# nirschl-lab/stain2stain

Measured on AMD Instinct MI355X. Metric: paired 256x256 stain tiles/sec (full CFM optimisation step), higher is better.
Workload: dtype bf16

## Files before the change

include/stain2stain_hip.h:

```cpp
#ifndef STAIN2STAIN_HIP_H
#define STAIN2STAIN_HIP_H

#ifdef __cplusplus
extern "C" {
#endif

#define S2S_OK 0
#define S2S_ERR_SHAPE (-1)
#define S2S_ERR_ALIGN (-2)
#define S2S_ERR_DTYPE (-3)
#define S2S_ERR_LAUNCH (-4)
#define S2S_ERR_NULL (-5)

#define S2S_BF16 0
#define S2S_F32 1

int s2s_conv3x3_stat_blocks(int dtype, int B, int H, int W, int Cout);
int s2s_conv3x3_nhwc(int dtype, const void* x0, int ld0, int c0, const void* x1, int ld1, int c1,
                     const void* w_packed, const float* bias, void* y, int ldy, float* stat_part,
                     const float* ep_scale, const float* ep_shift, int relu, int B, int H, int W, int Cout,
                     void* stream);

int s2s_conv3x3_ksplit(int dtype, int B, int H, int W, int Cout, int cin);
int s2s_conv3x3_nhwc_k(int dtype, const void* x0, int ld0, int c0, const void* x1, int ld1, int c1,
                       const void* w_packed, const float* bias, void* y, int ldy, float* stat_part,
                       const float* ep_scale, const float* ep_shift, int relu, float* kwork, int B, int H, int W,
                       int Cout, void* stream);
int s2s_conv3x3_stat_rows(int dtype, int B, int H, int W, int Cout, int c0, int c1, int ld0, int ld1, int has_bias);
int s2s_conv3x3_staged(int dtype, int B, int H, int W, int Cout, int c0, int c1, int ld0, int ld1, int ldy, int stats);
int s2s_conv3x3_family(int dtype, int B, int H, int W, int Cout, int c0, int c1, int ld0, int ld1, int ldy, int has_bias,
                       int has_affine, int stats, int stat_rows, int kwork);
int s2s_conv3x3_nhwc_s(int dtype, const void* x0, int ld0, int c0, const void* x1, int ld1, int c1, const void* w_packed,
                       const float* bias, void* y, int ldy, float* stat_part, int stat_rows, const float* ep_scale,
                       const float* ep_shift, int relu, float* kwork, int B, int H, int W, int Cout, void* stream);
int s2s_debug_conv_clock(long* out_host, int n);

int s2s_conv3x3_wgrad_splits(int dtype, int B, int H, int W, int Cin, int Cout);
int s2s_conv3x3_wgrad_nhwc(int dtype, const void* dy, int lddy, int Cout, const void* x0, int ld0, int c0,
                           const void* x1, int ld1, int c1, float* part, float* grad_oihw, int accumulate,
                           int B, int H, int W, void* stream);
int s2s_conv3x3_wgrad_phase(int dtype, const void* dy, int lddy, int Cout, const void* x0, int ld0, int c0,
                            const void* x1, int ld1, int c1, float* part, float* grad_oihw, int accumulate,
                            int B, int H, int W, int phases, void* stream);

int s2s_stem_stat_blocks(int B, int H, int W);
int s2s_stem_conv3x3_fwd(int dtype, const float* x_nchw, const float* w_oihw, const float* bias, void* y, int ldy,
                         float* stat_part, int B, int H, int W, int Cin, int Cout, void* stream);
int s2s_stem_wgrad_blocks(int B, int H, int W);
int s2s_stem_conv3x3_wgrad(int dtype, const void* dy, int lddy, const float* x_nchw, float* part, float* dw_oihw,
                           float* dbias, int accumulate, int B, int H, int W, int Cin, int Cout, void* stream);
int s2s_head_conv1x1_fwd(int dtype, const void* x, int ldx, const float* w, const float* bias, float* y_nchw, int B,
                         int H, int W, int C, int Cout, void* stream);
int s2s_head_wgrad_blocks(int B, int H, int W);
int s2s_head_conv1x1_bwd(int dtype, const float* dy_nchw, const void* x, int ldx, const float* w, void* dx, int lddx,
                         float* part, float* dw, float* dbias, int accumulate, int B, int H, int W, int C, int Cout,
                         void* stream);

int s2s_head_loss_blocks(int B, int H, int W);
int s2s_head_loss_fused(int dtype, const void* x, int ldx, const float* w, const float* bias, const float* u_nchw,
                        float* v_nchw, void* dx, int lddx, float grad_scale, float* part, double* lpart, float* dw,
                        float* dbias, float* loss, int accumulate, int B, int H, int W, int C, int Cout, void* stream);

int s2s_tail_blocks(int B, int H, int W);
int s2s_tail_fwd_loss(int dtype, const void* raw, int ldx, const float* scale, const float* shift, const float* mean,
                      const float* invstd, const float* w, const float* bias, const float* u_nchw, float* v_nchw,
                      float* g_nchw, float grad_scale, float* part, double* lpart, float* bnwork, float* dw,
                      float* dbias, float* loss, float* dgamma, float* dbeta, float* conv_dbias, int accumulate, int B,
                      int H, int W, int C, int Cout, void* stream);
int s2s_tail_bwd_apply(int dtype, const void* raw, int ldx, const float* g_nchw, const float* w, const float* scale,
                       const float* shift, const float* mean, const float* invstd, const float* gamma,
                       const float* bnwork, void* dx, int lddx, int B, int H, int W, int C, int Cout, void* stream);

int s2s_bn_finalize(const float* part, int nblk, int C, long count, const float* gamma, const float* beta,
                    float* running_mean, float* running_var, long* num_batches_tracked, float momentum, float eps,
                    float* mean, float* invstd, float* scale, float* shift, void* stream);
int s2s_bn_finalize_b(const float* part, int nblk, int C, long count, const float* gamma, const float* beta,
                      float* running_mean, float* running_var, long* num_batches_tracked, float momentum, float eps,
                      float* mean, float* invstd, float* scale, float* shift, const float* conv_bias, void* stream);
int s2s_bn_eval_prepare(int C, const float* gamma, const float* beta, const float* running_mean,
                        const float* running_var, float eps, float* scale, float* shift, void* stream);
int s2s_bn_relu_apply(int dtype, const void* x, int ldx, const float* scale, const float* shift, void* y, int ldy,
                      void* pool, int ldp, int B, int H, int W, int C, void* stream);
int s2s_maxpool2(int dtype, const void* x, int ldx, void* pool, int ldp, int B, int H, int W, int C, void* stream);
int s2s_bn_bwd_blocks(int B, int H, int W, int C);
int s2s_bn_relu_bwd(int dtype, const void* g1, int ldg1, const void* gp, int ldgp, const float* scale,
                    const float* shift, const void* x, int ldx, const float* mean, const float* invstd, const float* gamma, float* dgamma,
                    float* dbeta, float* dbias_conv, int accumulate, void* dx, int lddx, float* work, int B, int H,
                    int W, int C, void* stream);
int s2s_bn_partial_sums(const float* part, int nblk, int C, float* sums, void* stream);
int s2s_bn_relu_bwd_phase(int dtype, const void* g1, int ldg1, const void* gp, int ldgp, const float* scale,
                          const float* shift, const void* x, int ldx, const float* mean, const float* invstd,
                          const float* gamma, float* dgamma, float* dbeta, float* dbias_conv, int accumulate, void* dx,
                          int lddx, float* work, int B, int H, int W, int C, long count_total, int phases, void* stream);

int s2s_upsample2x_bilinear_ac_fwd(int dtype, const void* x, int ldx, const float* bias_nc, void* y, int ldy, int B,
                                   int Hin, int Win, int Hout, int Wout, int C, void* stream);
int s2s_upsample2x_bilinear_ac_bwd(int dtype, const void* dy, int lddy, void* dx, int lddx, int B, int Hin, int Win,
                                   int Hout, int Wout, int C, void* stream);
int s2s_upsample2x_bilinear_ac_bwd_ref(int dtype, const void* dy, int lddy, void* dx, int lddx, int B, int Hin,
                                       int Win, int Hout, int Wout, int C, void* stream);
int s2s_upsample2x_bwd_family(int lddy, int lddx, int B, int Hin, int Win, int Hout, int Wout, int C, int reference);
int s2s_pixel_sum(int dtype, const void* x, int ldx, float* out_nc, int B, int HW, int C, int accumulate,
                  void* stream);

int s2s_time_embedding(const float* t, float* out, int B, int dim, void* stream);
int s2s_linear_fwd(const float* x, const float* w, const float* bias, float* y, int B, int K, int N, void* stream);
int s2s_linear_bwd(const float* dy, const float* x, const float* w, float* dx, float* dw, float* db, int accumulate,
                   int B, int K, int N, void* stream);
int s2s_silu_fwd(const float* h, float* a, int n, void* stream);
int s2s_silu_bwd(const float* h, const float* da, float* dh, int n, void* stream);
int s2s_cfm_sample(const float* x0, const float* x1, const float* t, const float* eps, float sigma, float* xt,
                   float* ut, int B, long per_sample, void* stream);
int s2s_mse_loss(const float* v, const float* u, float* dv, float grad_scale, float* loss, double* work, long count,
                 void* stream);
int s2s_ode_error_norm(const float* e, const float* y0, const float* y1, float atol, float rtol, float* out,
                       double* work, long n, void* stream);
int s2s_axpy(float* x, const float* y, float a, long n, void* stream);
int s2s_dp_partials(long n);
int s2s_dp_init(int phase, const float* y, const float* k1, const float* fa, double* state, double* part, float* out,
                float* t_out, int* status, float atol, float rtol, int B, long n, void* stream);
int s2s_dp_stage(int i, const float* y, const float* k1, const float* k2, const float* k3, const float* k4,
                 const float* k5, const float* k6, const double* state, float* out, float* t_out, int B, long n,
                 void* stream);
int s2s_dp_error(const float* k1, const float* k2, const float* k3, const float* k4, const float* k5, const float* k6,
                 const float* k7, const float* y, const float* y_new, const double* state, double* part, float atol,
                 float rtol, int B, long n, void* stream);
int s2s_dp_control(double* state, const double* part, int* status, int max_steps, int B, long n, void* stream);
int s2s_dp_commit(float* y, const float* y_new, float* k1, const float* k7, const double* state, int B, long n,
                  void* stream);
int s2s_rk_stage(const float* x, const float* k1, const float* k2, const float* k3, float c1, float c2, float c3, int nk,
                 float* out, float* t_out, const float* table, const int* counter, int stages, int stage, int table_len,
                 int B, long n, void* stream);
int s2s_rk_combine(float* x, const float* k1, const float* k2, const float* k3, const float* k4, float c1, float c2,
                   float c3, float c4, int nk, int* counter, int B, long n, void* stream);
int s2s_fill_f32(float* x, float v, long n, void* stream);
int s2s_euler_tick(float* t, int n, const float* table, int* counter, void* stream);

int s2s_adam_step(float* p, const float* g, float* m, float* v, long n, int step, float lr, float beta1, float beta2,
                  float eps, float weight_decay, float grad_scale, void* stream);
int s2s_adam_step_dev(float* p, const float* g, float* m, float* v, long n, const float* hyper, void* stream);
long s2s_adam_multi_blocks(long n);
int s2s_adam_multi(const void* desc, int ntensors, long total, int step, float lr, float beta1, float beta2, float eps,
                   float weight_decay, float grad_scale, void* stream);
int s2s_adam_ema_step(float* p, const float* g, float* m, float* v, float* ema, long n, int step, float lr, float beta1,
                      float beta2, float eps, float weight_decay, float grad_scale, float ema_weight, void* stream);
int s2s_adam_ema_step_dev(float* p, const float* g, float* m, float* v, float* ema, long n, const float* hyper,
                          const float* ema_weight, void* stream);
long s2s_ema_multi_blocks(long n);
int s2s_ema_multi(const void* desc, int ntensors, long total, const float* weight, void* stream);
long s2s_pack_conv3x3_fwd_elems(int Cout, int Cin);
long s2s_pack_conv3x3_dgrad_elems(int Cout, int Cin);
int s2s_pack_conv3x3(int dtype, const float* w_oihw, void* w_fwd, void* w_dgrad, int Cout, int Cin, void* stream);
int s2s_pack_conv3x3_batched(int dtype, const void* desc, int nlayers, long total, void* stream);
int s2s_nchw_to_nhwc(int dtype, const float* x_nchw, void* y, int ldy, int B, int C, int H, int W, void* stream);
int s2s_nhwc_to_nchw(int dtype, const void* x, int ldx, float* y_nchw, int accumulate, int B, int C, int H, int W,
                     void* stream);

int s2s_paired_crop_flip_normalize(const void* src_u8, const void* tgt_u8, const int* params, float* out_src,
                                   float* out_tgt, int B, int Hs, int Ws, int S, void* stream);
int s2s_pil_resize_bilinear_normalize(const void* src_u8, void* tmp_u8, const int* bounds_h, const int* kk_h,
                                      int ksize_h, const int* bounds_v, const int* kk_v, int ksize_v, void* out_u8,
                                      float* out_f, int B, int Hs, int Ws, int Ho, int Wo, void* stream);

int s2s_region_gather(const void* img_u8, long pitch, int H, int W, int band_top, int band_h, const int* origins,
                      float* out, int B, int T, void* stream);
int s2s_region_blend(const float* tiles, int c0, const float* tiles1, int c1, const int* origins, int n, int T,
                     int overlap, float* acc, int band_rows, int H, int W, int r0, int r1, void* stream);
int s2s_region_finalize(float* acc, int band_rows, int W, int C, int r0, int r1, void* out_u8, long pitch_u8,
                        float* out_f, long pitch_f, int out_top, void* stream);

int s2s_region_tissue_count(const void* img_u8, long pitch, int H, int W, int band_top, int band_h, const int* origins,
                            int n, int T, int white, int black, int* counts, void* stream);
int s2s_region_skip_weight(const int* origins, int n, int T, int overlap, float* ws, int band_rows, int H, int W,
                           int r0, int r1, void* stream);
int s2s_region_finalize_mixed(float* acc, float* ws, int band_rows, int W, int C, int r0, int r1, const void* src_u8,
                              long src_pitch, int src_top, void* out_u8, long pitch_u8, float* out_f, long pitch_f,
                              int out_top, void* stream);

int s2s_seg_loss(const float* z, const float* g, float* dz, float* out, double* work, long n, float smooth,
// ... 186 lines not shown
```

stain2stain_amd/csrc/resample.hip:

```cpp
#include "common.h"
#include <stdlib.h>

namespace {

struct Axis {
  int i0, i1;
  float w0, w1;
};

__device__ __forceinline__ Axis ac_axis(int dst, int n_in, float scale) {
  Axis a;
  const float src = scale * (float)dst;
  a.i0 = (int)src;
  if (a.i0 > n_in - 1) a.i0 = n_in - 1;
  a.i1 = a.i0 + (a.i0 < n_in - 1 ? 1 : 0);
  a.w1 = src - (float)a.i0;
  a.w0 = 1.f - a.w1;
  return a;
}

__device__ __forceinline__ int rs_pcb(int C) {
  int p = 1;
  while (p < 32 && p * 8 < C) p <<= 1;
  return p;
}

template <typename T, bool BIAS>
__global__ __launch_bounds__(256) void upsample2x_fwd_kernel(const T* __restrict__ x, int ldx,
                                                             const float* __restrict__ bias, T* __restrict__ y,
                                                             int ldy, int B, int Hin, int Win, int Hout, int Wout,
                                                             int padT, int padL, int C, int band) {
  const int cp = C >> 3;
  const int Hu = 2 * Hin, Wu = 2 * Win;
  const float sh = Hu > 1 ? (float)(Hin - 1) / (float)(Hu - 1) : 0.f;
  const float sw = Wu > 1 ? (float)(Win - 1) / (float)(Wu - 1) : 0.f;
  const int PCB = rs_pcb(C), WL = 256 / PCB;
  const int pc = threadIdx.x & (PCB - 1), slot = threadIdx.x / PCB;
  const int nrows = B * Hout;
  for (int row0 = blockIdx.x * band; row0 < nrows; row0 += gridDim.x * band)
  for (int row = row0; row < row0 + band && row < nrows; ++row) {
    const int n = row / Hout, oy = row - n * Hout;
    const int uy = oy - padT;
    const bool row_in = uy >= 0 && uy < Hu;
    const Axis ay = ac_axis(row_in ? uy : 0, Hin, sh);
    const T* const r0 = x + ((long)n * Hin + ay.i0) * Win * ldx;
    const T* const r1 = x + ((long)n * Hin + ay.i1) * Win * ldx;
    T* const yr = y + (long)row * Wout * ldy;
    for (int pb = 0; pb < cp; pb += PCB) {
      const int c8 = (pb + pc) * 8;
      if (pb + pc >= cp) continue;
      float bv[8];
#pragma unroll
      for (int k = 0; k < 8; ++k) bv[k] = BIAS ? bias[(long)n * C + c8 + k] : 0.f;
      for (int ox = slot; ox < Wout; ox += WL) {
        const int ux = ox - padL;
        f32x8 o;
        if (!row_in || ux < 0 || ux >= Wu) {
#pragma unroll
          for (int k = 0; k < 8; ++k) o.v[k] = 0.f;
        } else {
          const Axis ax = ac_axis(ux, Win, sw);
          const int o0 = ax.i0 * ldx + c8, o1 = ax.i1 * ldx + c8;
          const f32x8 v00 = load8(r0 + o0), v01 = load8(r0 + o1), v10 = load8(r1 + o0), v11 = load8(r1 + o1);
#pragma unroll
          for (int k = 0; k < 8; ++k) {
            const float b = bv[k];
            o.v[k] = ay.w0 * (ax.w0 * (v00.v[k] + b) + ax.w1 * (v01.v[k] + b)) +
                     ay.w1 * (ax.w0 * (v10.v[k] + b) + ax.w1 * (v11.v[k] + b));
          }
        }
        store8(yr + ox * ldy + c8, o);
      }
    }
  }
}

template <typename T>
__global__ void upsample2x_bwd_kernel(const T* __restrict__ dy, int lddy, T* __restrict__ dx, int lddx, int B,
                                      int Hin, int Win, int Hout, int Wout, int padT, int padL, int C) {
  const int cp = C >> 3;
  const int Hu = 2 * Hin, Wu = 2 * Win;
  const float sh = Hu > 1 ? (float)(Hin - 1) / (float)(Hu - 1) : 0.f;
  const float sw = Wu > 1 ? (float)(Win - 1) / (float)(Wu - 1) : 0.f;
  const int total = B * Hin * Win * cp;
  for (int i = blockIdx.x * blockDim.x + threadIdx.x; i < total; i += gridDim.x * blockDim.x) {
    const int t0 = i / cp, c8 = (i - t0 * cp) * 8;
    const int t1 = t0 / Win, ix = t0 - t1 * Win;
    const int n = t1 / Hin, iy = t1 - n * Hin;
    int y_lo, y_hi, x_lo, x_hi;
    if (Hin == 1) { y_lo = 0; y_hi = Hu - 1; }
    else {
      y_lo = (int)floorf((float)(iy - 1) / sh) - 1; y_hi = (int)ceilf((float)(iy + 1) / sh) + 1;
      if (y_lo < 0) y_lo = 0;
      if (y_hi > Hu - 1) y_hi = Hu - 1;
    }
    if (Win == 1) { x_lo = 0; x_hi = Wu - 1; }
    else {
      x_lo = (int)floorf((float)(ix - 1) / sw) - 1; x_hi = (int)ceilf((float)(ix + 1) / sw) + 1;
      if (x_lo < 0) x_lo = 0;
      if (x_hi > Wu - 1) x_hi = Wu - 1;
    }
    constexpr int NSLOT = 12;
    float wxs[NSLOT];
#pragma unroll
    for (int j = 0; j < NSLOT; ++j) {
      const int ux = x_lo + j;
      float wx = 0.f;
      if (ux <= x_hi) {
        const Axis ax = ac_axis(ux, Win, sw);
        if (ax.i0 == ix) wx += ax.w0;
        if (ax.i1 == ix) wx += ax.w1;
        const int ox = ux + padL;
        if (ox < 0 || ox >= Wout) wx = 0.f;
      }
      wxs[j] = wx;
    }
    f32x8 acc;
#pragma unroll
    for (int k = 0; k < 8; ++k) acc.v[k] = 0.f;
    for (int uy = y_lo; uy <= y_hi; ++uy) {
      const Axis ay = ac_axis(uy, Hin, sh);
      float wy = 0.f;
      if (ay.i0 == iy) wy += ay.w0;
      if (ay.i1 == iy) wy += ay.w1;
      const int oy = uy + padT;
      if (wy == 0.f || oy < 0 || oy >= Hout) continue;
      const T* const rowp = dy + (((long)n * Hout + oy) * Wout + x_lo + padL) * lddy + c8;
#pragma unroll
      for (int j = 0; j < NSLOT; ++j) {
        if (wxs[j] == 0.f) continue;
        const f32x8 g = load8(rowp + (long)j * lddy);
        const float w = wy * wxs[j];
#pragma unroll
        for (int k = 0; k < 8; ++k) acc.v[k] += w * g.v[k];
      }
    }
    store8(dx + (((long)n * Hin + iy) * Win + ix) * lddx + c8, acc);
  }
}

__device__ __forceinline__ float ac_weight_of(int dst, int n_in, float scale, int src_index) {
  const Axis a = ac_axis(dst, n_in, scale);
  return (a.i0 == src_index ? a.w0 : 0.f) + (a.i1 == src_index ? a.w1 : 0.f);
}

template <typename T>
__global__ void upsample2x_bwd_win_kernel(const T* __restrict__ dy, int lddy, T* __restrict__ dx, int lddx, int B,
                                          int Hin, int Win, int Hout, int Wout, int padT, int padL, int C) {
  const int cp = C >> 3;
  const int Hu = 2 * Hin, Wu = 2 * Win;
  const float sh = (float)(Hin - 1) / (float)(Hu - 1), sw = (float)(Win - 1) / (float)(Wu - 1);
// ... 87 lines not shown
  if (piece >= cp) return;
  const int c8 = piece * 8;

  float wyA[4], wyB[4];
  const T* rowp[6];
#pragma unroll
  for (int j = 0; j < 6; ++j) {
    const int uy = 2 * iy0 - 1 + j;
    const bool in = uy >= 0 && uy <= Hu - 1;
    if (j < 4) wyA[j] = in ? ac_weight_of(uy, Hin, sh, iy0) : 0.f;
    if (j >= 2) wyB[j - 2] = in ? ac_weight_of(uy, Hin, sh, iy0 + 1) : 0.f;
    int oy = uy + padT;
    oy = oy < 0 ? 0 : (oy > Hout - 1 ? Hout - 1 : oy);
    rowp[j] = dy + ((long)n * Hout + oy) * Wout * lddy;
  }
  T* const dr0 = dx + ((long)n * Hin + iy0) * Win * lddx + c8;
  T* const dr1 = dr0 + (long)Win * lddx;

#pragma unroll 1
  for (int px = slot; px < WP; px += WL) {
    const int ix0 = min(2 * px, Win - 2);
    float wxA[4], wxB[4];
    int off[6];
#pragma unroll
    for (int m = 0; m < 6; ++m) {
      const int ux = 2 * ix0 - 1 + m;
      const bool in = ux >= 0 && ux <= Wu - 1;
      if (m < 4) wxA[m] = in ? ac_weight_of(ux, Win, sw, ix0) : 0.f;
      if (m >= 2) wxB[m - 2] = in ? ac_weight_of(ux, Win, sw, ix0 + 1) : 0.f;
      int ox = ux + padL;
      ox = ox < 0 ? 0 : (ox > Wout - 1 ? Wout - 1 : ox);
      off[m] = ox * lddy + c8;
    }
    f32x8 a00, a01, a10, a11;
#pragma unroll
    for (int k = 0; k < 8; ++k) a00.v[k] = a01.v[k] = a10.v[k] = a11.v[k] = 0.f;
#pragma unroll
    for (int j = 0; j < 6; ++j) {
      Raw8<T> cur[6];
#pragma unroll
      for (int m = 0; m < 6; ++m) cur[m] = load_raw8(rowp[j] + off[m]);
      f32x8 g[6];
#pragma unroll
      for (int m = 0; m < 6; ++m) g[m] = widen8(cur[m]);
      if (j < 4) {
#pragma unroll
        for (int m = 0; m < 4; ++m) {
          const float w = wyA[j] * wxA[m];
#pragma unroll
          for (int k = 0; k < 8; ++k) a00.v[k] = fmaf(w, g[m].v[k], a00.v[k]);
        }
#pragma unroll
        for (int m = 0; m < 4; ++m) {
          const float w = wyA[j] * wxB[m];
#pragma unroll
          for (int k = 0; k < 8; ++k) a01.v[k] = fmaf(w, g[m + 2].v[k], a01.v[k]);
        }
      }
      if (j >= 2) {
#pragma unroll
        for (int m = 0; m < 4; ++m) {
          const float w = wyB[j - 2] * wxA[m];
#pragma unroll
          for (int k = 0; k < 8; ++k) a10.v[k] = fmaf(w, g[m].v[k], a10.v[k]);
        }
#pragma unroll
        for (int m = 0; m < 4; ++m) {
          const float w = wyB[j - 2] * wxB[m];
#pragma unroll
          for (int k = 0; k < 8; ++k) a11.v[k] = fmaf(w, g[m + 2].v[k], a11.v[k]);
        }
      }
      if (j < 4) { pin8(a00); pin8(a01); }
      if (j >= 2) { pin8(a10); pin8(a11); }
      __builtin_amdgcn_sched_barrier(0);
    }
    store8(dr0 + ix0 * lddx, a00);
    store8(dr0 + (ix0 + 1) * lddx, a01);
    store8(dr1 + ix0 * lddx, a10);
    store8(dr1 + (ix0 + 1) * lddx, a11);
  }
}

template <typename T>
__global__ void pixel_sum_kernel(const T* __restrict__ x, int ldx, float* __restrict__ out, int HW, int C,
                                 int accumulate) {
  const int n = blockIdx.y;
  const int c = blockIdx.x * 64 + (threadIdx.x & 63);
  const int rg = threadIdx.x >> 6;
  float s = 0.f;
  if (c < C) {
    constexpr int U = 16;
    const T* const xp = x + (long)n * HW * ldx + c;
    int p = rg;
    for (; p + 4 * (U - 1) < HW; p += 4 * U) {
      float v[U];
#pragma unroll
      for (int u = 0; u < U; ++u) v[u] = to_f32(xp[(long)(p + 4 * u) * ldx]);
#pragma unroll
      for (int u = 0; u < U; ++u) s += v[u];
    }
    for (; p < HW; p += 4) s += to_f32(xp[(long)p * ldx]);
  }
  __shared__ float red[4][64];
  red[rg][threadIdx.x & 63] = s;
  __syncthreads();
  if (rg == 0 && c < C) {
    s = red[0][threadIdx.x] + red[1][threadIdx.x] + red[2][threadIdx.x] + red[3][threadIdx.x];
    out[(long)n * C + c] = accumulate ? out[(long)n * C + c] + s : s;
  }
}

inline int ew_grid(long total) {
  long b = (total + 255) / 256;
  if (b > 8192) b = 8192;
  if (b < 1) b = 1;
  return (int)b;
}

}

extern "C" int s2s_upsample2x_bilinear_ac_fwd(int dtype, const void* x, int ldx, const float* bias_nc, void* y,
                                              int ldy, int B, int Hin, int Win, int Hout, int Wout, int C,
                                              void* stream) {
  if (!x || !y) return S2S_ERR_NULL;
  if (B <= 0 || Hin <= 0 || Win <= 0 || C <= 0 || (C % 8) || (ldx % 8) || (ldy % 8)) return S2S_ERR_SHAPE;
  if (Hout < 2 * Hin || Wout < 2 * Win) return S2S_ERR_SHAPE;
  const int padT = (Hout - 2 * Hin) / 2, padL = (Wout - 2 * Win) / 2;
  if ((long)Win * ldx >= (1L << 31) || (long)Wout * ldy >= (1L << 31) || (long)B * Hout >= (1L << 31))
    return S2S_ERR_SHAPE;
  hipStream_t s = (hipStream_t)stream;
  const long rows = (long)B * Hout;
  static const int band_env = [] { const char* e = getenv("S2S_UP_BAND"); return e ? atoi(e) : 0; }();
  const int band = band_env > 0 ? band_env : (rows >= 4096 ? 4 : rows >= 2048 ? 2 : 1);
  const long nwg = (rows + band - 1) / band;
  const dim3 grid((unsigned)(nwg < 65535 * 4 ? nwg : 65535 * 4));
#define S2S_UP(TT, BB)                                                                                          \
  hipLaunchKernelGGL((upsample2x_fwd_kernel<TT, BB>), grid, dim3(256), 0, s, (const TT*)x, ldx, bias_nc, (TT*)y, \
                     ldy, B, Hin, Win, Hout, Wout, padT, padL, C, band)
  if (dtype == S2S_BF16) { if (bias_nc) S2S_UP(bf16_t, true); else S2S_UP(bf16_t, false); }
  else if (dtype == S2S_F32) { if (bias_nc) S2S_UP(float, true); else S2S_UP(float, false); }
  else return S2S_ERR_DTYPE;
#undef S2S_UP
  S2S_LAUNCH_CHECK();
  return S2S_OK;
}

namespace {

enum UpBwdFamily { kUpBwdGather = 0, kUpBwdWindow = 1, kUpBwdQuad = 2 };

int upsample2x_bwd_family(int lddy, int lddx, int B, int Hin, int Win, int Wout, int C, bool reference) {
  if (!(Hin > 3 && Win > 3)) return kUpBwdGather;
  const long nwork = (long)B * ((Hin + 1) / 2);
  const bool quad = !reference && Hin <= 4096 && Win <= 4096 && (long)Wout * lddy < (1L << 31) &&
                    (long)Win * lddx < (1L << 31) && nwork * cdiv(C / 8, 32) < (1L << 31);
  return quad ? kUpBwdQuad : kUpBwdWindow;
}

int upsample2x_bwd_launch(int dtype, const void* dy, int lddy, void* dx, int lddx, int B, int Hin, int Win, int Hout,
                          int Wout, int C, void* stream, bool reference) {
  if (!dy || !dx) return S2S_ERR_NULL;
  if (B <= 0 || Hin <= 0 || Win <= 0 || C <= 0 || (C % 8) || (lddy % 8) || (lddx % 8)) return S2S_ERR_SHAPE;
  if (Hout < 2 * Hin || Wout < 2 * Win) return S2S_ERR_SHAPE;
  const int padT = (Hout - 2 * Hin) / 2, padL = (Wout - 2 * Win) / 2;
  const long total = (long)B * Hin * Win * (C / 8);
  if (total >= (1L << 31) - (1L << 22)) return S2S_ERR_SHAPE;
  hipStream_t s = (hipStream_t)stream;
  const dim3 grid(ew_grid(total));
  if (dtype != S2S_BF16 && dtype != S2S_F32) return S2S_ERR_DTYPE;
  const int family = upsample2x_bwd_family(lddy, lddx, B, Hin, Win, Wout, C, reference);
  const bool win = family != kUpBwdGather;
  const int nchunk = cdiv(C / 8, 32);
  const long nwork = (long)B * ((Hin + 1) / 2);
  if (family == kUpBwdQuad) {
    const dim3 qgrid((unsigned)(nwork * nchunk));
    if (dtype == S2S_BF16)
      hipLaunchKernelGGL(upsample2x_bwd_quad_kernel<bf16_t>, qgrid, dim3(256), 0, s, (const bf16_t*)dy, lddy,
                         (bf16_t*)dx, lddx, B, Hin, Win, Hout, Wout, padT, padL, C, (int)nwork);
    else
      hipLaunchKernelGGL(upsample2x_bwd_quad_kernel<float>, qgrid, dim3(256), 0, s, (const float*)dy, lddy, (float*)dx,
                         lddx, B, Hin, Win, Hout, Wout, padT, padL, C, (int)nwork);
    S2S_LAUNCH_CHECK();
    return S2S_OK;
  }
#define S2S_UPB(KERN, TT)                                                                                           \
  hipLaunchKernelGGL(KERN<TT>, grid, dim3(256), 0, s, (const TT*)dy, lddy, (TT*)dx, lddx, B, Hin, Win, Hout, Wout,   \
                     padT, padL, C)
  if (dtype == S2S_BF16) { if (win) S2S_UPB(upsample2x_bwd_win_kernel, bf16_t); else S2S_UPB(upsample2x_bwd_kernel, bf16_t); }
  else { if (win) S2S_UPB(upsample2x_bwd_win_kernel, float); else S2S_UPB(upsample2x_bwd_kernel, float); }
#undef S2S_UPB
  S2S_LAUNCH_CHECK();
  return S2S_OK;
}

}

extern "C" int s2s_upsample2x_bilinear_ac_bwd(int dtype, const void* dy, int lddy, void* dx, int lddx, int B, int Hin,
                                              int Win, int Hout, int Wout, int C, void* stream) {
  return upsample2x_bwd_launch(dtype, dy, lddy, dx, lddx, B, Hin, Win, Hout, Wout, C, stream, false);
}

extern "C" int s2s_upsample2x_bilinear_ac_bwd_ref(int dtype, const void* dy, int lddy, void* dx, int lddx, int B,
                                                  int Hin, int Win, int Hout, int Wout, int C, void* stream) {
  return upsample2x_bwd_launch(dtype, dy, lddy, dx, lddx, B, Hin, Win, Hout, Wout, C, stream, true);
}

extern "C" int s2s_upsample2x_bwd_family(int lddy, int lddx, int B, int Hin, int Win, int Hout, int Wout, int C,
                                         int reference) {
  if (B <= 0 || Hin <= 0 || Win <= 0 || C <= 0 || (C % 8) || (lddy % 8) || (lddx % 8)) return S2S_ERR_SHAPE;
  if (Hout < 2 * Hin || Wout < 2 * Win) return S2S_ERR_SHAPE;
  if ((long)B * Hin * Win * (C / 8) >= (1L << 31) - (1L << 22)) return S2S_ERR_SHAPE;
  return upsample2x_bwd_family(lddy, lddx, B, Hin, Win, Wout, C, reference != 0);
}

extern "C" int s2s_pixel_sum(int dtype, const void* x, int ldx, float* out_nc, int B, int HW, int C, int accumulate,
                             void* stream) {
  if (!x || !out_nc) return S2S_ERR_NULL;
  if (B <= 0 || HW <= 0 || C <= 0) return S2S_ERR_SHAPE;
  hipStream_t s = (hipStream_t)stream;
  dim3 grid(cdiv(C, 64), B);
  if (dtype == S2S_BF16)
    hipLaunchKernelGGL(pixel_sum_kernel<bf16_t>, grid, dim3(256), 0, s, (const bf16_t*)x, ldx, out_nc, HW, C, accumulate);
  else if (dtype == S2S_F32)
    hipLaunchKernelGGL(pixel_sum_kernel<float>, grid, dim3(256), 0, s, (const float*)x, ldx, out_nc, HW, C, accumulate);
  else return S2S_ERR_DTYPE;
  S2S_LAUNCH_CHECK();
  return S2S_OK;
// ... 2 lines not shown
```

stain2stain_amd/ops.py:

```python
from __future__ import annotations

import contextlib
import ctypes
import os
import sys
from typing import Optional, Tuple

import torch

from . import _native

BF16, F32 = 0, 1


def _dt(t: torch.Tensor) -> int:
    if t.dtype == torch.bfloat16:
        return BF16
    if t.dtype == torch.float32:
        return F32
    raise RuntimeError(f"stain2stain_amd: unsupported activation dtype {t.dtype}")


_raw_stream = getattr(torch._C, "_cuda_getCurrentRawStream", None)
_raw_device = getattr(torch._C, "_cuda_getDevice", None)
# ... 427 lines not shown
                                _f32(running_var), 0 if num_batches is None else num_batches.data_ptr(), momentum, eps,
                                out[0].data_ptr(), out[1].data_ptr(), out[2].data_ptr(), out[3].data_ptr(),
                                _f32(conv_bias), _stream())
    _native.check(rc, "bn_finalize")
    return out


def bn_partial_sums(stat: torch.Tensor) -> torch.Tensor:
    _, C, nblk = stat.shape
    sums = torch.empty((2, C), dtype=torch.float32, device=stat.device)
    _native.check(_L().s2s_bn_partial_sums(_f32(stat), nblk, C, _f32(sums), _stream()), "bn_partial_sums")
    return sums


def bn_eval_prepare(gamma, beta, rmean, rvar, eps: float = 1e-5):
    C = gamma.numel()
    out = torch.empty((2, C), dtype=torch.float32, device=gamma.device)
    rc = _L().s2s_bn_eval_prepare(C, _f32(gamma), _f32(beta), _f32(rmean), _f32(rvar), eps, out[0].data_ptr(),
                                  out[1].data_ptr(), _stream())
    _native.check(rc, "bn_eval_prepare")
    return out


@_timed("bn_relu_apply")
def bn_relu_apply(x: torch.Tensor, scale: torch.Tensor, shift: torch.Tensor, out: Optional[torch.Tensor] = None,
                  pool: Optional[torch.Tensor] = None, want_pool: bool = False):
    B, H, W, C = x.shape
    px, ldx = _nhwc(x)
    if out is None:
        out = torch.empty((B, H, W, C), dtype=x.dtype, device=x.device)
    py, ldy = _nhwc(out)
    pp, ldp = 0, 8
    if want_pool and pool is None:
        pool = torch.empty((B, H // 2, W // 2, C), dtype=x.dtype, device=x.device)
    if pool is not None:
        pp, ldp = _nhwc(pool)
    rc = _L().s2s_bn_relu_apply(_dt(x), px, ldx, _f32(scale), _f32(shift), py, ldy, pp, ldp, B, H, W, C, _stream())
    _native.check(rc, "bn_relu_apply")
    return out, pool


@_timed("maxpool2")
def maxpool2(x: torch.Tensor) -> torch.Tensor:
    B, H, W, C = x.shape
    px, ldx = _nhwc(x)
    pool = torch.empty((B, H // 2, W // 2, C), dtype=x.dtype, device=x.device)
    rc = _L().s2s_maxpool2(_dt(x), px, ldx, pool.data_ptr(), C, B, H, W, C, _stream())
    _native.check(rc, "maxpool2")
    return pool


@_timed("bn_relu_bwd")
def bn_relu_bwd(g1: Optional[torch.Tensor], gp: Optional[torch.Tensor], x: torch.Tensor,
                stats: torch.Tensor, gamma: torch.Tensor, dgamma: torch.Tensor, dbeta: torch.Tensor,
                dbias_conv: Optional[torch.Tensor], accumulate: bool = False, exchange=None,
                count_total: Optional[int] = None) -> torch.Tensor:
    B, H, W, C = x.shape
    px, ldx = _nhwc(x)
    p1, ld1 = (0, 8) if g1 is None else _nhwc(g1)
    p2, ld2 = (0, 8) if gp is None else _nhwc(gp)
    dx = torch.empty((B, H, W, C), dtype=x.dtype, device=x.device)
    nb = _L().s2s_bn_bwd_blocks(B, H, W, C)
    work = torch.empty((4 * nb * C + 2 * C,), dtype=torch.float32, device=x.device)
    if exchange is not None:
        for phase in (1, 2):
            rc = _L().s2s_bn_relu_bwd_phase(_dt(x), p1, ld1, p2, ld2, stats[2].data_ptr(), stats[3].data_ptr(), px, ldx,
                                            stats[0].data_ptr(), stats[1].data_ptr(),
                                            _f32(gamma), _f32(dgamma), _f32(dbeta), _f32(dbias_conv), int(accumulate),
                                            dx.data_ptr(), C, _f32(work), B, H, W, C,
                                            int(count_total if count_total is not None else B * H * W), phase, _stream())
            _native.check(rc, "bn_relu_bwd")
            if phase == 1:
                exchange(work[4 * nb * C:])
        return dx
    rc = _L().s2s_bn_relu_bwd(_dt(x), p1, ld1, p2, ld2, stats[2].data_ptr(), stats[3].data_ptr(), px, ldx,
                              stats[0].data_ptr(), stats[1].data_ptr(),
                              _f32(gamma), _f32(dgamma), _f32(dbeta), _f32(dbias_conv), int(accumulate),
                              dx.data_ptr(), C, _f32(work), B, H, W, C, _stream())
    _native.check(rc, "bn_relu_bwd")
    return dx


@_timed("upsample2x_fwd")
def upsample2x_fwd(x: torch.Tensor, out: torch.Tensor, bias_nc: Optional[torch.Tensor] = None) -> None:
    B, Hin, Win, C = x.shape
    _, Hout, Wout, Co = out.shape
    if Co != C or out.dtype != x.dtype:
        raise RuntimeError("stain2stain_amd: upsample output slice mismatch")
    px, ldx = _nhwc(x)
    py, ldy = _nhwc(out)
    rc = _L().s2s_upsample2x_bilinear_ac_fwd(_dt(x), px, ldx, _f32(bias_nc), py, ldy, B, Hin, Win, Hout, Wout, C,
                                             _stream())
    _native.check(rc, "upsample2x_fwd")


@_timed("upsample2x_bwd")
def upsample2x_bwd(dy: torch.Tensor, hin: int, win: int, _reference: bool = False) -> torch.Tensor:
    B, Hout, Wout, C = dy.shape
    pdy, lddy = _nhwc(dy)
    dx = torch.empty((B, hin, win, C), dtype=dy.dtype, device=dy.device)
    fn = _L().s2s_upsample2x_bilinear_ac_bwd_ref if _reference else _L().s2s_upsample2x_bilinear_ac_bwd
    rc = fn(_dt(dy), pdy, lddy, dx.data_ptr(), C, B, hin, win, Hout, Wout, C, _stream())
    _native.check(rc, "upsample2x_bwd")
    return dx


def upsample2x_bwd_family(dy: torch.Tensor, hin: int, win: int, _reference: bool = False) -> int:
    B, Hout, Wout, C = dy.shape
    rc = _L().s2s_upsample2x_bwd_family(dy.stride(2), C, B, hin, win, Hout, Wout, C, int(_reference))
    if rc < 0:
        _native.check(rc, "upsample2x_bwd_family")
    return rc


def pixel_sum(x: torch.Tensor) -> torch.Tensor:
    B, H, W, C = x.shape
    px, ldx = _nhwc(x)
    out = torch.empty((B, C), dtype=torch.float32, device=x.device)
    rc = _L().s2s_pixel_sum(_dt(x), px, ldx, _f32(out), B, H * W, C, 0, _stream())
    _native.check(rc, "pixel_sum")
    return out


def time_embedding(t: torch.Tensor, dim: int) -> torch.Tensor:
    t = t.reshape(-1).to(torch.float32).contiguous()
    out = torch.empty((t.numel(), dim), dtype=torch.float32, device=t.device)
    _native.check(_L().s2s_time_embedding(_f32(t), _f32(out), t.numel(), dim, _stream()), "time_embedding")
    return out


def linear_fwd(x: torch.Tensor, w: torch.Tensor, b: Optional[torch.Tensor]) -> torch.Tensor:
    B, K = x.shape
    N = w.shape[0]
    y = torch.empty((B, N), dtype=torch.float32, device=x.device)
    _native.check(_L().s2s_linear_fwd(_f32(x), _f32(w), _f32(b), _f32(y), B, K, N, _stream()), "linear_fwd")
    return y


def linear_bwd(dy: torch.Tensor, x: torch.Tensor, w: torch.Tensor, dw: torch.Tensor, db: Optional[torch.Tensor],
               need_dx: bool = True, accumulate: bool = False) -> Optional[torch.Tensor]:
    B, K = x.shape
    N = w.shape[0]
    dx = torch.empty((B, K), dtype=torch.float32, device=x.device) if need_dx else None
    _native.check(_L().s2s_linear_bwd(_f32(dy), _f32(x), _f32(w), _f32(dx), _f32(dw), _f32(db), int(accumulate), B, K,
                                      N, _stream()), "linear_bwd")
    return dx


def silu_fwd(h: torch.Tensor) -> torch.Tensor:
    a = torch.empty_like(h)
    _native.check(_L().s2s_silu_fwd(_f32(h), _f32(a), h.numel(), _stream()), "silu_fwd")
    return a


def silu_bwd(h: torch.Tensor, da: torch.Tensor) -> torch.Tensor:
    dh = torch.empty_like(h)
    _native.check(_L().s2s_silu_bwd(_f32(h), _f32(da), _f32(dh), h.numel(), _stream()), "silu_bwd")
    return dh


@_timed("cfm_sample")
def cfm_sample(x0: torch.Tensor, x1: torch.Tensor, t: torch.Tensor, sigma: float = 0.0,
               eps: Optional[torch.Tensor] = None):
    xt = torch.empty_like(x0)
    ut = torch.empty_like(x0)
    B = x0.shape[0]
    _native.check(_L().s2s_cfm_sample(_f32(x0), _f32(x1), _f32(t), _f32(eps), float(sigma), _f32(xt), _f32(ut), B,
                                      x0.numel() // B, _stream()), "cfm_sample")
    return xt, ut


@_timed("mse_loss")
def mse_loss(v: torch.Tensor, u: torch.Tensor, want_grad: bool = True, grad_scale: float = 1.0):
    loss = torch.empty((), dtype=torch.float32, device=v.device)
    dv = torch.empty_like(v) if want_grad else None
    work = torch.empty((1024,), dtype=torch.float64, device=v.device)
# ... 1182 lines not shown
```

Before: 2264.

## Add windowed bilinear upsample forward kernel reusing input rows across output pairs

Adds a new forward upsample kernel in which each thread owns one input column and a band of input rows. It mixes each input row horizontally once, keeps three mixed rows in registers and emits two output rows and two output columns per input position, writing padding only at the edges. This is meant to cut the redundant input loads and horizontal interpolation that the row-per-output kernel repeats for every output pixel. The grid is remapped across 8 interleaved classes, and launch bounds allow higher occupancy for bf16 without bias. In exchange it adds a fallback path for irregular row pairs, heavier register use, and fma-based weight arithmetic that can change rounding slightly.

```diff
diff --git a/include/stain2stain_hip.h b/include/stain2stain_hip.h
--- a/include/stain2stain_hip.h
+++ b/include/stain2stain_hip.h
@@ -95,6 +95,9 @@
 
 int s2s_upsample2x_bilinear_ac_fwd(int dtype, const void* x, int ldx, const float* bias_nc, void* y, int ldy, int B,
                                    int Hin, int Win, int Hout, int Wout, int C, void* stream);
+int s2s_upsample2x_bilinear_ac_fwd_ref(int dtype, const void* x, int ldx, const float* bias_nc, void* y, int ldy, int B,
+                                       int Hin, int Win, int Hout, int Wout, int C, void* stream);
+int s2s_upsample2x_fwd_family(int ldx, int ldy, int B, int Hin, int Win, int Hout, int Wout, int C, int reference);
 int s2s_upsample2x_bilinear_ac_bwd(int dtype, const void* dy, int lddy, void* dx, int lddx, int B, int Hin, int Win,
                                    int Hout, int Wout, int C, void* stream);
 int s2s_upsample2x_bilinear_ac_bwd_ref(int dtype, const void* dy, int lddy, void* dx, int lddx, int B, int Hin,
diff --git a/stain2stain_amd/csrc/resample.hip b/stain2stain_amd/csrc/resample.hip
--- a/stain2stain_amd/csrc/resample.hip
+++ b/stain2stain_amd/csrc/resample.hip
@@ -19,7 +19,24 @@
   return a;
 }
 
-__device__ __forceinline__ int rs_pcb(int C) {
+__device__ __forceinline__ Axis ac_axis_fwd(int dst, int n_in, float scale) {
+  Axis a = ac_axis(dst, n_in, scale);
+  a.w1 = __builtin_fmaf(scale, (float)dst, -(float)a.i0);
+  a.w0 = 1.f - a.w1;
+  return a;
+}
+
+__device__ __forceinline__ float up_mix2(float w0, float p, float w1, float q, int k) {
+  return (k & 1) ? __builtin_fmaf(w0, p, w1 * q) : __builtin_fmaf(w1, q, w0 * p);
+}
+__device__ __forceinline__ float up_row_mix(const Axis& ax, float v0, float v1, float b, int k) {
+  return up_mix2(ax.w0, v0 + b, ax.w1, v1 + b, k);
+}
+__device__ __forceinline__ float up_col_mix(const Axis& ay, float h0, float h1, int k) {
+  return up_mix2(ay.w0, h0, ay.w1, h1, k);
+}
+
+__host__ __device__ __forceinline__ int rs_pcb(int C) {
   int p = 1;
   while (p < 32 && p * 8 < C) p <<= 1;
   return p;
@@ -42,7 +59,7 @@
     const int n = row / Hout, oy = row - n * Hout;
     const int uy = oy - padT;
     const bool row_in = uy >= 0 && uy < Hu;
-    const Axis ay = ac_axis(row_in ? uy : 0, Hin, sh);
+    const Axis ay = ac_axis_fwd(row_in ? uy : 0, Hin, sh);
     const T* const r0 = x + ((long)n * Hin + ay.i0) * Win * ldx;
     const T* const r1 = x + ((long)n * Hin + ay.i1) * Win * ldx;
     T* const yr = y + (long)row * Wout * ldy;
@@ -59,14 +76,13 @@
 #pragma unroll
           for (int k = 0; k < 8; ++k) o.v[k] = 0.f;
         } else {
-          const Axis ax = ac_axis(ux, Win, sw);
+          const Axis ax = ac_axis_fwd(ux, Win, sw);
           const int o0 = ax.i0 * ldx + c8, o1 = ax.i1 * ldx + c8;
           const f32x8 v00 = load8(r0 + o0), v01 = load8(r0 + o1), v10 = load8(r1 + o0), v11 = load8(r1 + o1);
 #pragma unroll
           for (int k = 0; k < 8; ++k) {
             const float b = bv[k];
-            o.v[k] = ay.w0 * (ax.w0 * (v00.v[k] + b) + ax.w1 * (v01.v[k] + b)) +
-                     ay.w1 * (ax.w0 * (v10.v[k] + b) + ax.w1 * (v11.v[k] + b));
+            o.v[k] = up_col_mix(ay, up_row_mix(ax, v00.v[k], v01.v[k], b, k), up_row_mix(ax, v10.v[k], v11.v[k], b, k), k);
           }
         }
         store8(yr + ox * ldy + c8, o);
@@ -320,6 +336,117 @@
   }
 }
 
+__device__ __forceinline__ bool up_usual_pair(const Axis (&ay)[2], int a) {
+  const bool u = ay[0].i0 == a - 1 && ay[0].i1 == a && ay[1].i0 == a && ay[1].i1 == a + 1;
+  return __builtin_amdgcn_readfirstlane((int)u) != 0;
+}
+
+template <typename T>
+struct UpTaps { Raw8<T> t[2][2]; };
+struct UpMix2 { f32x8 e[2]; };
+
+template <typename T, bool BIAS>
+__global__ __launch_bounds__(256, sizeof(T) == 2 && !BIAS ? 4 : 2) void upsample2x_fwd_win_kernel(
+    const T* __restrict__ x, int ldx, const float* __restrict__ bias, T* __restrict__ y, int ldy, int B, int Hin, int Win,
+    int Hout, int Wout, int padT, int padL, int C, int band, int nband, int ncol, int nwork) {
+  constexpr unsigned ES = sizeof(T);
+  const int cp = C >> 3;
+  const int Hu = 2 * Hin, Wu = 2 * Win;
+  const float sh = (float)(Hin - 1) / (float)(Hu - 1), sw = (float)(Win - 1) / (float)(Wu - 1);
+  const int PCB = rs_pcb(C), WL = 256 / PCB;
+  const int pc = threadIdx.x & (PCB - 1), slot = threadIdx.x / PCB;
+  const int nwg = gridDim.x, q = nwg >> 3, r = nwg & 7, cls = blockIdx.x & 7;
+  const int wgid = (cls < r ? cls * (q + 1) : r * (q + 1) + (cls - r) * q) + (blockIdx.x >> 3);
+  const int chunk = wgid / nwork;
+  int work = wgid - chunk * nwork;
+  const int cg = work % ncol; work /= ncol;
+  const int bi = work % nband, n = work / nband;
+  const int a0 = bi * band, a1 = min(a0 + band, Hin);
+  const int sx = cg * WL + slot, piece = chunk * PCB + pc;
+  if (sx >= Win || piece >= cp) return;
+  const int c8 = piece * 8;
+
+  float bv[8];
+#pragma unroll
+  for (int k = 0; k < 8; ++k) bv[k] = BIAS ? bias[(long)n * C + c8 + k] : 0.f;
+
+  const Axis ax[2] = {ac_axis_fwd(2 * sx, Win, sw), ac_axis_fwd(2 * sx + 1, Win, sw)};
+  const unsigned off[2][2] = {{(unsigned)(ax[0].i0 * ldx + c8) * ES, (unsigned)(ax[0].i1 * ldx + c8) * ES},
+                              {(unsigned)(ax[1].i0 * ldx + c8) * ES, (unsigned)(ax[1].i1 * ldx + c8) * ES}};
+  const int ox0 = padL + 2 * sx;
+  const unsigned yo[2] = {(unsigned)(ox0 * ldy + c8) * ES, (unsigned)((ox0 + 1) * ldy + c8) * ES};
+  const char* const xn = reinterpret_cast<const char*>(x + (long)n * Hin * Win * ldx);
+  char* const yn = reinterpret_cast<char*>(y + (long)n * Hout * Wout * ldy);
+  const long xrow = (long)Win * ldx * ES, yrow = (long)Wout * ldy * ES;
+
+  auto load_row = [&](int iy) {
+    const char* const rp = xn + min(max(iy, 0), Hin - 1) * xrow;
+    UpTaps<T> w;
+#pragma unroll
+    for (int e = 0; e < 2; ++e)
+#pragma unroll
+      for (int t = 0; t < 2; ++t) w.t[e][t] = load_raw8(reinterpret_cast<const T*>(rp + off[e][t]));
+    return w;
+  };
+  auto mix_row = [&](const UpTaps<T>& w) {
+    UpMix2 m;
+#pragma unroll
+    for (int e = 0; e < 2; ++e) {
+      const f32x8 v0 = widen8(w.t[e][0]), v1 = widen8(w.t[e][1]);
+#pragma unroll
+      for (int k = 0; k < 8; ++k) m.e[e].v[k] = up_row_mix(ax[e], v0.v[k], v1.v[k], bv[k], k);
+    }
+    return m;
+  };
+  auto put_row = [&](char* yr, const Axis& ay, const UpMix2& top, const UpMix2& bot) {
+#pragma unroll
+    for (int f = 0; f < 2; ++f) {
+      f32x8 o;
+#pragma unroll
+      for (int k = 0; k < 8; ++k) o.v[k] = up_col_mix(ay, top.e[f].v[k], bot.e[f].v[k], k);
+      store8(reinterpret_cast<T*>(yr + yo[f]), o);
+    }
+  };
+
+  UpMix2 m0 = mix_row(load_row(a0 - 1)), m1 = mix_row(load_row(a0)), m2 = mix_row(load_row(a0 + 1));
+#pragma unroll 1
+  for (int a = a0; a < a1; ++a) {
+    const UpTaps<T> nx = load_row(min(a + 2, a1));
+    const Axis ay[2] = {ac_axis_fwd(2 * a, Hin, sh), ac_axis_fwd(2 * a + 1, Hin, sh)};
+    if (up_usual_pair(ay, a)) {
+      char* const yr = yn + (padT + 2 * a) * yrow;
+      put_row(yr, ay[0], m0, m1);
+      put_row(yr + yrow, ay[1], m1, m2);
+    }
+    m0 = m1;
+    m1 = m2;
+    m2 = mix_row(nx);
+  }
+#pragma unroll 1
+  for (int a = a0; a < a1; ++a) {
+    const Axis ay[2] = {ac_axis_fwd(2 * a, Hin, sh), ac_axis_fwd(2 * a + 1, Hin, sh)};
+    if (up_usual_pair(ay, a)) continue;
+#pragma unroll 1
+    for (int e = 0; e < 2; ++e) {
+      const Axis ae = ac_axis_fwd(2 * a + e, Hin, sh);
+      const UpMix2 top = mix_row(load_row(ae.i0)), bot = mix_row(load_row(ae.i1));
+      put_row(yn + (padT + 2 * a + e) * yrow, ae, top, bot);
+    }
+  }
+
+  const int zl = sx == 0 ? 0 : ox0, zr = sx == Win - 1 ? Wout : ox0 + 2;
+  const int ry0 = a0 == 0 ? 0 : padT + 2 * a0, ry1 = a1 == Hin ? Hout : padT + 2 * a1;
+  f32x8 zero;
+#pragma unroll
+  for (int k = 0; k < 8; ++k) zero.v[k] = 0.f;
+  for (int oy = ry0; oy < ry1; ++oy) {
+    const bool pad_row = oy < padT || oy >= padT + Hu;
+    char* const yr = yn + oy * yrow;
+    for (int ox = zl; ox < zr; ++ox)
+      if (pad_row || ox < ox0 || ox >= ox0 + 2) store8(reinterpret_cast<T*>(yr + (unsigned)(ox * ldy + c8) * ES), zero);
+  }
+}
+
 template <typename T>
 __global__ void pixel_sum_kernel(const T* __restrict__ x, int ldx, float* __restrict__ out, int HW, int C,
                                  int accumulate) {
@@ -358,30 +485,89 @@
 
 }
 
-extern "C" int s2s_upsample2x_bilinear_ac_fwd(int dtype, const void* x, int ldx, const float* bias_nc, void* y,
-                                              int ldy, int B, int Hin, int Win, int Hout, int Wout, int C,
-                                              void* stream) {
-  if (!x || !y) return S2S_ERR_NULL;
+namespace {
+
+enum UpFwdFamily { kUpFwdRows = 0, kUpFwdWindow = 1 };
+
+int up_band_env() {
+  static const int band_env = [] { const char* e = getenv("S2S_UP_BAND"); return e ? atoi(e) : 0; }();
+  return band_env;
+}
+
+int upsample2x_fwd_band(int B, int Hin, int Win, int C) {
+  if (up_band_env() > 0) return up_band_env();
+  const long per_band = (long)B * cdiv(Win, 256 / rs_pcb(C)) * cdiv(C / 8, 32);
+  return per_band * cdiv(Hin, 8) >= 2048 ? 8 : 4;
+}
+
+int upsample2x_fwd_family(int ldx, int ldy, int B, int Hin, int Win, int Wout, int C, bool reference) {
+  if (reference || Hin < 2 || Win < 2 || Hin > 4096 || Win > 4096) return kUpFwdRows;
+  if ((long)Win * ldx >= (1L << 29) || (long)Wout * ldy >= (1L << 29)) return kUpFwdRows;
+  const long nwg = (long)B * cdiv(Hin, upsample2x_fwd_band(B, Hin, Win, C)) * cdiv(Win, 256 / rs_pcb(C)) *
+                   cdiv(C / 8, 32);
+  return nwg < (1L << 31) ? kUpFwdWindow : kUpFwdRows;
+}
+
+int upsample2x_fwd_check(int ldx, int ldy, int B, int Hin, int Win, int Hout, int Wout, int C) {
   if (B <= 0 || Hin <= 0 || Win <= 0 || C <= 0 || (C % 8) || (ldx % 8) || (ldy % 8)) return S2S_ERR_SHAPE;
   if (Hout < 2 * Hin || Wout < 2 * Win) return S2S_ERR_SHAPE;
-  const int padT = (Hout - 2 * Hin) / 2, padL = (Wout - 2 * Win) / 2;
   if ((long)Win * ldx >= (1L << 31) || (long)Wout * ldy >= (1L << 31) || (long)B * Hout >= (1L << 31))
     return S2S_ERR_SHAPE;
+  return S2S_OK;
+}
+
+int upsample2x_fwd_launch(int dtype, const void* x, int ldx, const float* bias_nc, void* y, int ldy, int B, int Hin,
+                          int Win, int Hout, int Wout, int C, void* stream, bool reference) {
+  if (!x || !y) return S2S_ERR_NULL;
+  if (int rc = upsample2x_fwd_check(ldx, ldy, B, Hin, Win, Hout, Wout, C)) return rc;
+  if (dtype != S2S_BF16 && dtype != S2S_F32) return S2S_ERR_DTYPE;
+  const int padT = (Hout - 2 * Hin) / 2, padL = (Wout - 2 * Win) / 2;
   hipStream_t s = (hipStream_t)stream;
+  if (upsample2x_fwd_family(ldx, ldy, B, Hin, Win, Wout, C, reference) == kUpFwdWindow) {
+    const int band = upsample2x_fwd_band(B, Hin, Win, C), nband = cdiv(Hin, band);
+    const int ncol = cdiv(Win, 256 / rs_pcb(C)), nwork = B * nband * ncol;
+    const dim3 wgrid((unsigned)((long)nwork * cdiv(C / 8, 32)));
+#define S2S_UPW(TT, BB)                                                                                              \
+  hipLaunchKernelGGL((upsample2x_fwd_win_kernel<TT, BB>), wgrid, dim3(256), 0, s, (const TT*)x, ldx, bias_nc, (TT*)y, \
+                     ldy, B, Hin, Win, Hout, Wout, padT, padL, C, band, nband, ncol, nwork)
+    if (dtype == S2S_BF16) { if (bias_nc) S2S_UPW(bf16_t, true); else S2S_UPW(bf16_t, false); }
+    else { if (bias_nc) S2S_UPW(float, true); else S2S_UPW(float, false); }
+#undef S2S_UPW
+    S2S_LAUNCH_CHECK();
+    return S2S_OK;
+  }
   const long rows = (long)B * Hout;
-  static const int band_env = [] { const char* e = getenv("S2S_UP_BAND"); return e ? atoi(e) : 0; }();
-  const int band = band_env > 0 ? band_env : (rows >= 4096 ? 4 : rows >= 2048 ? 2 : 1);
+  const int band = up_band_env() > 0 ? up_band_env() : (rows >= 4096 ? 4 : rows >= 2048 ? 2 : 1);
   const long nwg = (rows + band - 1) / band;
   const dim3 grid((unsigned)(nwg < 65535 * 4 ? nwg : 65535 * 4));
 #define S2S_UP(TT, BB)                                                                                          \
   hipLaunchKernelGGL((upsample2x_fwd_kernel<TT, BB>), grid, dim3(256), 0, s, (const TT*)x, ldx, bias_nc, (TT*)y, \
                      ldy, B, Hin, Win, Hout, Wout, padT, padL, C, band)
   if (dtype == S2S_BF16) { if (bias_nc) S2S_UP(bf16_t, true); else S2S_UP(bf16_t, false); }
-  else if (dtype == S2S_F32) { if (bias_nc) S2S_UP(float, true); else S2S_UP(float, false); }
-  else return S2S_ERR_DTYPE;
+  else { if (bias_nc) S2S_UP(float, true); else S2S_UP(float, false); }
 #undef S2S_UP
   S2S_LAUNCH_CHECK();
   return S2S_OK;
+}
+
+}
+
+extern "C" int s2s_upsample2x_bilinear_ac_fwd(int dtype, const void* x, int ldx, const float* bias_nc, void* y,
+                                              int ldy, int B, int Hin, int Win, int Hout, int Wout, int C,
+                                              void* stream) {
+  return upsample2x_fwd_launch(dtype, x, ldx, bias_nc, y, ldy, B, Hin, Win, Hout, Wout, C, stream, false);
+}
+
+extern "C" int s2s_upsample2x_bilinear_ac_fwd_ref(int dtype, const void* x, int ldx, const float* bias_nc, void* y,
+                                                  int ldy, int B, int Hin, int Win, int Hout, int Wout, int C,
+                                                  void* stream) {
+  return upsample2x_fwd_launch(dtype, x, ldx, bias_nc, y, ldy, B, Hin, Win, Hout, Wout, C, stream, true);
+}
+
+extern "C" int s2s_upsample2x_fwd_family(int ldx, int ldy, int B, int Hin, int Win, int Hout, int Wout, int C,
+                                         int reference) {
+  if (int rc = upsample2x_fwd_check(ldx, ldy, B, Hin, Win, Hout, Wout, C)) return rc;
+  return upsample2x_fwd_family(ldx, ldy, B, Hin, Win, Wout, C, reference != 0);
 }
 
 namespace {
diff --git a/stain2stain_amd/ops.py b/stain2stain_amd/ops.py
--- a/stain2stain_amd/ops.py
+++ b/stain2stain_amd/ops.py
@@ -533,16 +533,26 @@
 
 
 @_timed("upsample2x_fwd")
-def upsample2x_fwd(x: torch.Tensor, out: torch.Tensor, bias_nc: Optional[torch.Tensor] = None) -> None:
+def upsample2x_fwd(x: torch.Tensor, out: torch.Tensor, bias_nc: Optional[torch.Tensor] = None,
+                   _reference: bool = False) -> None:
     B, Hin, Win, C = x.shape
     _, Hout, Wout, Co = out.shape
     if Co != C or out.dtype != x.dtype:
         raise RuntimeError("stain2stain_amd: upsample output slice mismatch")
     px, ldx = _nhwc(x)
     py, ldy = _nhwc(out)
-    rc = _L().s2s_upsample2x_bilinear_ac_fwd(_dt(x), px, ldx, _f32(bias_nc), py, ldy, B, Hin, Win, Hout, Wout, C,
-                                             _stream())
+    fn = _L().s2s_upsample2x_bilinear_ac_fwd_ref if _reference else _L().s2s_upsample2x_bilinear_ac_fwd
+    rc = fn(_dt(x), px, ldx, _f32(bias_nc), py, ldy, B, Hin, Win, Hout, Wout, C, _stream())
     _native.check(rc, "upsample2x_fwd")
+
+
+def upsample2x_fwd_family(x: torch.Tensor, out: torch.Tensor, _reference: bool = False) -> int:
+    B, Hin, Win, C = x.shape
+    _, Hout, Wout, _ = out.shape
+    rc = _L().s2s_upsample2x_fwd_family(_nhwc(x)[1], _nhwc(out)[1], B, Hin, Win, Hout, Wout, C, int(_reference))
+    if rc < 0:
+        _native.check(rc, "upsample2x_fwd_family")
+    return rc
 
 
 @_timed("upsample2x_bwd")
```

Result: faster. 2324 (median of 6 runs) (+2.6%).
